# baldhat/yolov10-3D

Hardware: AMD Instinct MI355X
Metric: train_images_per_sec (higher is better)
Workload: dtype bf16

## Files before the change

yolov10-3d_amd/csrc/conv3x3_wgrad_tile.hip:

```cpp
#include "common.h"
#include <cstdlib>

namespace {

__device__ uint4 y3d_wg_zero_page[4];

struct WG3P {
  const void* x;
  const void* dy;
  float* slab;
  long xsb, xsh, xsw, dsw;
  int B, H, W;
  int Cg, Cn, G;
  int ntx, nty;
  int ntiles, tiles_per_split, nslab;
};

typedef __attribute__((ext_vector_type(8))) short s16x8_t;

template <int OFF>
__device__ __forceinline__ s16x4_t ds_tr16(unsigned a) {
  s16x4_t v;
#ifdef Y3D_WGP_NOLDS
  asm volatile("" : "=v"(v) : "v"(a));
  return v;
#endif
  asm volatile("ds_read_b64_tr_b16 %0, %1 offset:%2" : "=v"(v) : "v"(a), "n"(OFF));
  return v;
}
template <int N>
__device__ __forceinline__ void lds_wait(s16x4_t& a, s16x4_t& b, s16x4_t& c, s16x4_t& d) {
  asm volatile("s_waitcnt lgkmcnt(%4)" : "+v"(a), "+v"(b), "+v"(c), "+v"(d) : "n"(N));
}

template <int N>
__device__ __forceinline__ void lds_wait8(s16x4_t& a, s16x4_t& b, s16x4_t& c, s16x4_t& d, s16x4_t& e, s16x4_t& f, s16x4_t& g, s16x4_t& h) {
  asm volatile("s_waitcnt lgkmcnt(%8)" : "+v"(a), "+v"(b), "+v"(c), "+v"(d), "+v"(e), "+v"(f), "+v"(g), "+v"(h) : "n"(N));
}

template <int TH>
__global__ __launch_bounds__(512) void conv3x3_wgrad_tile_kernel(WG3P p) {
  typedef bf16_t T;
  constexpr int NT = 512;
  constexpr int NPX = TH * 16;
  constexpr int HWD = 18;
  constexpr int NPIXH = (TH + 2) * HWD;
  constexpr int DR = NPX * 16 / NT;
  constexpr int HCH = NPIXH * 8;
  constexpr int HR = (HCH + NT - 1) / NT;
  constexpr int DBYTES = NPX * 256, HBYTES = HR * NT * 16, SBYTES = DBYTES + HBYTES;
  extern __shared__ __attribute__((aligned(16))) char smem[];

  const int tid = threadIdx.x, lane = tid & 63, wave = tid >> 6;
  const int wi = wave >> 1, wj = wave & 1;
  const int g = blockIdx.z, split = blockIdx.y;
  const int slab_i = blockIdx.x % p.nslab, cot = blockIdx.x / p.nslab;
  const int c0 = cot * 128, ci0 = slab_i * 64;
  const T* __restrict__ X = (const T*)p.x;
  const T* __restrict__ D = (const T*)p.dy;
  const T* zero = (const T*)y3d_wg_zero_page;

  int d_row[DR], d_px[DR], d_c[DR];
#pragma unroll
  for (int rd = 0; rd < DR; ++rd) {
    int chunk = rd * NT + tid;
    int pp = chunk >> 4, s = chunk & 15;
    d_row[rd] = pp >> 4;
    d_px[rd] = pp & 15;
    d_c[rd] = (s ^ ((pp & 7) << 1)) * 8;
  }
  int h_y[HR], h_x[HR], h_c[HR];
#pragma unroll
  for (int rd = 0; rd < HR; ++rd) {
    int chunk = rd * NT + tid;
    int P = chunk >> 3, s = chunk & 7;
    h_y[rd] = chunk < HCH ? P / HWD : -100000;
    h_x[rd] = P - (P / HWD) * HWD;
    h_c[rd] = (s ^ (((h_x[rd] >> 1) & 3) << 1)) * 8;
  }
  auto issue = [&](int tile, int buf) {
    int tx = tile % p.ntx;
    int t2 = tile / p.ntx;
    int ty = t2 % p.nty;
    int b = t2 / p.nty;
    const int x0 = tx * 16, y0 = ty * TH;
    char* db = smem + buf * SBYTES;
    char* hb = db + DBYTES;
#pragma unroll
    for (int rd = 0; rd < DR; ++rd) {
      int xx = x0 + d_px[rd];
      bool ok = xx < p.W && c0 + d_c[rd] < p.Cn;
      const T* src = ok ? D + (((long)b * p.H + y0 + d_row[rd]) * p.W + xx) * p.dsw + (long)g * p.Cn + c0 + d_c[rd] : zero;
#ifndef Y3D_WGP_NODMA
      __builtin_amdgcn_global_load_lds((const __attribute__((address_space(1))) void*)src,
                                       (__attribute__((address_space(3))) void*)(db + (rd * NT + wave * 64) * 16), 16, 0, 0);
#else
      asm volatile("" ::"v"(src));
#endif
    }
#pragma unroll
    for (int rd = 0; rd < HR; ++rd) {
      if (rd * NT + tid < HCH) {
        int yy = y0 + h_y[rd] - 1, xx = x0 + h_x[rd] - 1;
        bool ok = yy >= 0 && yy < p.H && xx >= 0 && xx < p.W && ci0 + h_c[rd] < p.Cg;
        const T* src = ok ? X + (long)b * p.xsb + (long)yy * p.xsh + (long)xx * p.xsw + (long)g * p.Cg + ci0 + h_c[rd] : zero;
#ifndef Y3D_WGP_NODMA
        __builtin_amdgcn_global_load_lds((const __attribute__((address_space(1))) void*)src,
                                         (__attribute__((address_space(3))) void*)(hb + (rd * NT + wave * 64) * 16), 16, 0, 0);
#else
        asm volatile("" ::"v"(src));
#endif
      }
    }
  };

  f32x4_t acc[9][2][2];
#pragma unroll
  for (int t = 0; t < 9; ++t)
#pragma unroll
    for (int a = 0; a < 2; ++a)
#pragma unroll
      for (int c = 0; c < 2; ++c) acc[t][a][c] = (f32x4_t){0.f, 0.f, 0.f, 0.f};

  const int t_beg = split * p.tiles_per_split;
  const int t_end = min(p.ntiles, t_beg + p.tiles_per_split);
  const int grp = lane >> 4, li = lane & 15, qq = li >> 2, pp4 = li & 3;

  unsigned aoff[2], boff[3][2];
  {
    const int px8 = 4 * grp + qq;
#pragma unroll
    for (int mt = 0; mt < 2; ++mt) {
      const int cch = ((wi * 32 + mt * 16) >> 3) + (pp4 >> 1);
      aoff[mt] = px8 * 256 + ((cch ^ ((px8 & 7) << 1)) << 4) + (pp4 & 1) * 8;
    }
#pragma unroll
    for (int q = 0; q < 3; ++q)
#pragma unroll
      for (int nt = 0; nt < 2; ++nt) {
        const int x = px8 + q;
        const int cch = ((wj * 32 + nt * 16) >> 3) + (pp4 >> 1);
        boff[q][nt] = x * 128 + ((cch ^ (((x >> 1) & 3) << 1)) << 4) + (pp4 & 1) * 8;
      }
  }
  const unsigned smem_base = (unsigned)(size_t)(__attribute__((address_space(3))) const char*)smem;

  if (t_beg < t_end) issue(t_beg, 0);
  asm volatile("s_waitcnt vmcnt(0)" ::: "memory");
  __syncthreads();
  for (int tile = t_beg; tile < t_end; ++tile) {
    const int cur = (tile - t_beg) & 1;
    if (tile + 1 < t_end) issue(tile + 1, cur ^ 1);
#pragma unroll
    for (int ks = 0; ks < NPX / 32; ++ks) {
      bf16x8_t fa[2];
      s16x4_t va[2][2];
      const unsigned dks = smem_base + cur * SBYTES + ks * 8192;
      const unsigned hks = smem_base + cur * SBYTES + DBYTES + ks * (2 * HWD * 128);
#pragma unroll
      for (int mt = 0; mt < 2; ++mt) {
        va[mt][0] = ds_tr16<0>(dks + aoff[mt]);
        va[mt][1] = ds_tr16<4096>(dks + aoff[mt]);
      }
      s16x4_t vr[2][2][4];
      auto issue_q = [&](int q, int buf) {
#pragma unroll
        for (int nt = 0; nt < 2; ++nt) {
          const unsigned a = hks + boff[q][nt];
          vr[buf][nt][0] = ds_tr16<0>(a);
          vr[buf][nt][1] = ds_tr16<HWD * 128>(a);
          vr[buf][nt][2] = ds_tr16<2 * HWD * 128>(a);
          vr[buf][nt][3] = ds_tr16<3 * HWD * 128>(a);
        }
      };
      issue_q(0, 0);
      lds_wait<8>(va[0][0], va[0][1], va[1][0], va[1][1]);
#pragma unroll
      for (int mt = 0; mt < 2; ++mt) fa[mt] = __builtin_bit_cast(bf16x8_t, __builtin_shufflevector(va[mt][0], va[mt][1], 0, 1, 2, 3, 4, 5, 6, 7));
#pragma unroll
      for (int q = 0; q < 3; ++q) {
        const int cb = q & 1;
        if (q < 2) {
          issue_q(q + 1, cb ^ 1);
          lds_wait8<8>(vr[cb][0][0], vr[cb][0][1], vr[cb][0][2], vr[cb][0][3], vr[cb][1][0], vr[cb][1][1], vr[cb][1][2], vr[cb][1][3]);
        } else {
          lds_wait8<0>(vr[cb][0][0], vr[cb][0][1], vr[cb][0][2], vr[cb][0][3], vr[cb][1][0], vr[cb][1][1], vr[cb][1][2], vr[cb][1][3]);
        }
#pragma unroll
        for (int r = 0; r < 3; ++r) {
          bf16x8_t fb[2];
#pragma unroll
          for (int nt = 0; nt < 2; ++nt)
            fb[nt] = __builtin_bit_cast(bf16x8_t, __builtin_shufflevector(vr[cb][nt][r], vr[cb][nt][r + 1], 0, 1, 2, 3, 4, 5, 6, 7));
#pragma unroll
          for (int mt = 0; mt < 2; ++mt)
#pragma unroll
            for (int nt = 0; nt < 2; ++nt)
#ifndef Y3D_WGP_NOMFMA
              acc[r * 3 + q][mt][nt] = __builtin_amdgcn_mfma_f32_16x16x32_bf16(fa[mt], fb[nt], acc[r * 3 + q][mt][nt], 0, 0, 0);
#else
              asm volatile("" ::"v"(fa[mt]), "v"(fb[nt]));
#endif
        }
      }
    }
    asm volatile("s_waitcnt vmcnt(0)" ::: "memory");
    __syncthreads();
  }

  const int Ktot = 9 * p.Cg;
  float* slab = p.slab + ((long)split * p.G * p.Cn + (long)g * p.Cn) * Ktot;
#pragma unroll
  for (int tap = 0; tap < 9; ++tap)
#pragma unroll
    for (int mt = 0; mt < 2; ++mt)
#pragma unroll
      for (int nt = 0; nt < 2; ++nt) {
        int ci = ci0 + wj * 32 + nt * 16 + (lane & 15);
#pragma unroll
        for (int rg = 0; rg < 4; ++rg) {
          int co = c0 + wi * 32 + mt * 16 + (lane >> 4) * 4 + rg;
          if (co < p.Cn && ci < p.Cg) slab[(long)co * Ktot + tap * p.Cg + ci] = acc[tap][mt][nt][rg];
        }
      }
}

template <int TH>
int launch_wg(const WG3P& p, int nsplit, hipStream_t st) {
  constexpr int NPX = TH * 16;
  constexpr int HCH = (TH + 2) * 18 * 8;
  constexpr int HR = (HCH + 511) / 512;
  size_t sm = 2 * ((size_t)NPX * 256 + (size_t)HR * 512 * 16);
  static bool attr_set = false;
  if (!attr_set) {
    (void)hipFuncSetAttribute((const void*)conv3x3_wgrad_tile_kernel<TH>, hipFuncAttributeMaxDynamicSharedMemorySize, (int)sm);
    attr_set = true;
  }
  dim3 grid(p.nslab * cdiv(p.Cn, 128), nsplit, p.G);
  hipLaunchKernelGGL((conv3x3_wgrad_tile_kernel<TH>), grid, dim3(512), sm, st, p);
  Y3D_LAUNCH_CHECK();
  return Y3D_OK;
}

}

int y3d_wgrad_tile_height(int dtype, int H, int W, int Cg, int Cn, int kh, int kw, int stride, int pad) {
  if (dtype != Y3D_BF16 || kh != 3 || kw != 3 || stride != 1 || pad != 1) return 0;
  if (Cg % 16 != 0 || Cg < 64 || Cn % 8 != 0 || W < 8) return 0;
  if (H % 8 == 0) return 8;
  if (H % 4 == 0) return 4;
  return 0;
}

int y3d_wgrad_tile_splits(int th, int B, int H, int W, int Cg, int Cn, int G) {
  long ntiles = (long)B * (H / th) * cdiv(W, 16);
  long blocks = (long)cdiv(Cg, 64) * cdiv(Cn, 128) * G;
  const int target8 = 256;
  const long tgt = th == 8 ? target8 : 2 * target8;
  long want = tgt / blocks;
  if (want > ntiles) want = ntiles;
  long slab_bytes = (long)G * Cn * 9 * Cg * 4;
  long cap = (64L << 20) / slab_bytes;
  if (cap < 16) cap = 16;
  if (cap > 256) cap = 256;
  if (want > cap) want = cap;
  if (want < 1) want = 1;
  return (int)want;
}

int y3d_conv3x3_wgrad_tile_launch(int th, const void* x, long xsb, long xsh, long xsw, const void* dy, long dsw, int B, int H, int W, int Cg,
                                  int Cn, int G, float* slab, int nsplit, void* stream) {
  WG3P p;
  p.x = x; p.dy = dy; p.slab = slab;
  p.xsb = xsb; p.xsh = xsh; p.xsw = xsw; p.dsw = dsw;
  p.B = B; p.H = H; p.W = W; p.Cg = Cg; p.Cn = Cn; p.G = G;
  p.ntx = cdiv(W, 16); p.nty = H / th;
  p.ntiles = B * p.nty * p.ntx;
  p.tiles_per_split = cdiv(p.ntiles, nsplit);
  p.nslab = cdiv(Cg, 64);
  hipStream_t st = (hipStream_t)stream;
  if (th == 8) return launch_wg<8>(p, nsplit, st);
  return launch_wg<4>(p, nsplit, st);
}
```

yolov10-3d_amd/csrc/conv_gemm.hip:

```cpp
#include "common.h"
#include "conv_frag.h"
#include <cstdlib>

namespace {

struct ConvP {
  const void* x;
  const void* w;
  const float* bias;
  const float* scale;
  const float* shift;
  int act;
  void* y;
  float* part;
  long xsb, xsh, xsw;
  long ysw;
  int B, Hg, Wg;
  int Hq, Wq;
  int Cg, Cn, G;
  int kh, kw, stride, pad;
  int Ktot, Kpad;
  int M;
  int ntx, nty;
};
// ... 216 lines not shown
      for (int j = 0; j < 4; ++j) {
        float u = acc[a][b][j] + bv[j];
        if (p.scale) { u = u * sv[j] + hv[j]; if (p.act) u = silu_f(u); }
        v[j] = TT<T>::rnd(u);
        ssum[a][j] += v[j];
        ssq[a][j] += v[j] * v[j];
      }
      if (m < Mc) {
        T* dst = Y + opix * p.ysw + (long)g * p.Cn + co;
        if (co + 3 < p.Cn && ((p.Cn | p.ysw) & 3) == 0) {
          if (sizeof(T) == 2) {
            uint2 u;
            u.x = (unsigned)f2bf(v[0]) | ((unsigned)f2bf(v[1]) << 16);
            u.y = (unsigned)f2bf(v[2]) | ((unsigned)f2bf(v[3]) << 16);
            *(uint2*)dst = u;
          } else {
            *(float4*)dst = make_float4(v[0], v[1], v[2], v[3]);
          }
        } else {
#pragma unroll
          for (int j = 0; j < 4; ++j) if (co + j < p.Cn) TT<T>::st(dst + j, v[j]);
        }
      }
    }
  }
  if (p.part) {
    float* red = (float*)smem;
#pragma unroll
    for (int a = 0; a < TC; ++a)
#pragma unroll
      for (int j = 0; j < 4; ++j) {
        float s = wave_xor_sum16(ssum[a][j]);
        float q = wave_xor_sum16(ssq[a][j]);
        if (lp == 0) {
          int cl = wc * (BC / WC) + a * 16 + lc + j;
          red[(wp * BC + cl) * 2 + 0] = s;
          red[(wp * BC + cl) * 2 + 1] = q;
        }
      }
    __syncthreads();
    if (tid < BC && c0 + tid < p.Cn) {
      float s = 0.f, q = 0.f;
#pragma unroll
      for (int w = 0; w < WP; ++w) { s += red[(w * BC + tid) * 2]; q += red[(w * BC + tid) * 2 + 1]; }
      float* dst = p.part + ((long)tile_x * (p.G * p.Cn) + g * p.Cn + c0 + tid) * 2;
      dst[0] = s;
      dst[1] = q;
    }
  }
}

struct WgradP {
  const void* x;
  const void* dy;
  float* slab;
  long xsb, xsh, xsw;
  long dsw;
  int B, H, W, Ho, Wo;
  int Cg, Cn, G;
  int kh, kw, stride, pad;
  int Ktot, M, nsplit, chunk_px;
};

template <typename T, int W> struct TFrag;
template <int W> struct TFrag<bf16_t, W> {
  typedef bf16x8_t type;
  static constexpr int KSUB_PX = 32;
  static constexpr int PITCH = W * 2 + 32;
  __device__ static __forceinline__ type load(const char* tile, int i0, int k0, int lane) {
    int grp = lane >> 4, li = lane & 15;
    int q = li >> 2, pp = li & 3;
    const char* a0 = tile + (k0 + 4 * grp + q) * PITCH + (i0 + 4 * pp) * 2;
    s16x4_t lo = __builtin_amdgcn_ds_read_tr16_b64_v4i16((s16x4_t __attribute__((address_space(3)))*)(a0));
    s16x4_t hi = __builtin_amdgcn_ds_read_tr16_b64_v4i16((s16x4_t __attribute__((address_space(3)))*)(a0 + 16 * PITCH));
    typedef __attribute__((ext_vector_type(8))) short s16x8_t;
    s16x8_t v = __builtin_shufflevector(lo, hi, 0, 1, 2, 3, 4, 5, 6, 7);
    return __builtin_bit_cast(bf16x8_t, v);
  }
  __device__ static __forceinline__ f32x4_t mma(type a, type b, f32x4_t c) {
    return __builtin_amdgcn_mfma_f32_16x16x32_bf16(a, b, c, 0, 0, 0);
  }
};
template <int W> struct TFrag<float, W> {
  typedef float type;
  static constexpr int KSUB_PX = 4;
  static constexpr int PITCH = W * 4 + 64;
  __device__ static __forceinline__ type load(const char* tile, int i0, int k0, int lane) {
    return *(const float*)(tile + (k0 + (lane >> 4)) * PITCH + (i0 + (lane & 15)) * 4);
  }
  __device__ static __forceinline__ f32x4_t mma(type a, type b, f32x4_t c) {
    return __builtin_amdgcn_mfma_f32_16x16x4f32(a, b, c, 0, 0, 0);
  }
};

template <typename T, int WD, int WX>
__global__ __launch_bounds__(256) void conv_wgrad_kernel(WgradP p) {
  constexpr int CE = TT<T>::CE;
  constexpr int BPK = TT<T>::BKE;
  constexpr int PD = TFrag<T, WD>::PITCH, PX = TFrag<T, WX>::PITCH;
  constexpr int CPD = WD * sizeof(T) / 16, CPX = WX * sizeof(T) / 16;
  constexpr int ND = BPK * CPD / 256 > 0 ? BPK * CPD / 256 : 1;
  constexpr int NX = BPK * CPX / 256 > 0 ? BPK * CPX / 256 : 1;
  constexpr int TA = WD / 32, TB = WX / 32;
  extern __shared__ __attribute__((aligned(16))) char smem[];
  char* sD = smem;
  char* sX = smem + 2 * BPK * PD;

  const int tid = threadIdx.x, lane = tid & 63, wave = tid >> 6;
  const int wi = wave >> 1, wj = wave & 1;
  const int g = blockIdx.z % p.G;
  const int split = blockIdx.z / p.G;
  const int j0 = blockIdx.x * WX;
  const int i0 = blockIdx.y * WD;
  const T* __restrict__ X = (const T*)p.x;
  const T* __restrict__ D = (const T*)p.dy;

  const int mbeg = split * p.chunk_px;
  const int mend = min(p.M, mbeg + p.chunk_px);
  const int nsteps = (mend - mbeg + BPK - 1) / BPK;

  const int ccd = tid % CPD, rd0 = tid / CPD;
  const int ccx = tid % CPX, rx0 = tid / CPX;
  constexpr int RSD = 256 / CPD, RSX = 256 / CPX;
  const bool tdv = BPK * CPD >= 256 || tid < BPK * CPD, txv = BPK * CPX >= 256 || tid < BPK * CPX;
  const int kx = j0 + ccx * CE;
  const bool kx_ok = txv && kx < p.Ktot;
  int tap = 0, ci = 0, tr = 0, tq = 0;
  if (kx_ok) { tap = kx / p.Cg; ci = kx - tap * p.Cg; tr = tap / p.kw; tq = tap - tr * p.kw; }
  const int cd = i0 + ccd * CE;
  const bool cd_ok = tdv && cd < p.Cn;
  const int HW = p.Ho * p.Wo;

  uint4 rd[ND], rx[NX];
  int rb_[NX], rh_[NX], rw_[NX];
#pragma unroll
  for (int i = 0; i < NX; ++i) {
    int m = mbeg + rx0 + RSX * i;
    int b = m / HW;
    int rem = m - b * HW;
    rb_[i] = b;
    rh_[i] = rem / p.Wo;
    rw_[i] = rem - rh_[i] * p.Wo;
  }
  const T* dcol = D + (long)g * p.Cn + cd;
  const T* xcol = X + (long)g * p.Cg + ci + (long)(tr - p.pad) * p.xsh + (long)(tq - p.pad) * p.xsw;
  auto gload = [&](int st) {
#pragma unroll
    for (int i = 0; i < ND; ++i) {
      int m = mbeg + st * BPK + rd0 + RSD * i;
      uint4 vd = make_uint4(0, 0, 0, 0);
      if (m < mend && cd_ok) vd = *(const uint4*)(dcol + (long)m * p.dsw);
      rd[i] = vd;
    }
#pragma unroll
    for (int i = 0; i < NX; ++i) {
      int m = mbeg + st * BPK + rx0 + RSX * i;
      uint4 vx = make_uint4(0, 0, 0, 0);
      if (m < mend && kx_ok) {
        int hh = rh_[i] * p.stride - p.pad + tr, ww = rw_[i] * p.stride - p.pad + tq;
        if (hh >= 0 && ww >= 0 && hh < p.H && ww < p.W)
          vx = *(const uint4*)(xcol + (long)rb_[i] * p.xsb + (long)(rh_[i] * p.stride) * p.xsh + (long)(rw_[i] * p.stride) * p.xsw);
      }
      rx[i] = vx;
      rw_[i] += BPK;
      while (rw_[i] >= p.Wo) { rw_[i] -= p.Wo; ++rh_[i]; }
      while (rh_[i] >= p.Ho) { rh_[i] -= p.Ho; ++rb_[i]; }
    }
  };
  auto lstore = [&](int buf) {
    if (tdv) {
#pragma unroll
      for (int i = 0; i < ND; ++i) *(uint4*)(sD + buf * BPK * PD + (rd0 + RSD * i) * PD + ccd * 16) = rd[i];
    }
    if (txv) {
#pragma unroll
      for (int i = 0; i < NX; ++i) *(uint4*)(sX + buf * BPK * PX + (rx0 + RSX * i) * PX + ccx * 16) = rx[i];
    }
  };

  f32x4_t acc[TA][TB];
#pragma unroll
  for (int a = 0; a < TA; ++a)
#pragma unroll
    for (int b = 0; b < TB; ++b) acc[a][b] = (f32x4_t){0.f, 0.f, 0.f, 0.f};

  if (nsteps > 0) {
    gload(0);
    lstore(0);
  }
  __syncthreads();
  for (int st = 0; st < nsteps; ++st) {
    const int cur = st & 1;
    if (st + 1 < nsteps) gload(st + 1);
    const char* tD = sD + cur * BPK * PD;
    const char* tX = sX + cur * BPK * PX;
#pragma unroll
    for (int k0 = 0; k0 < BPK; k0 += TFrag<T, WD>::KSUB_PX) {
      typename TFrag<T, WD>::type fa[TA], fb[TB];
#pragma unroll
      for (int a = 0; a < TA; ++a) fa[a] = TFrag<T, WD>::load(tD, wi * (WD / 2) + a * 16, k0, lane);
#pragma unroll
      for (int b = 0; b < TB; ++b) fb[b] = TFrag<T, WX>::load(tX, wj * (WX / 2) + b * 16, k0, lane);
#pragma unroll
      for (int a = 0; a < TA; ++a)
#pragma unroll
        for (int b = 0; b < TB; ++b) acc[a][b] = TFrag<T, WD>::mma(fa[a], fb[b], acc[a][b]);
    }
    if (st + 1 < nsteps) lstore(cur ^ 1);
    __syncthreads();
  }
  float* slab = p.slab + ((long)split * p.G * p.Cn + (long)g * p.Cn) * p.Ktot;
#pragma unroll
  for (int a = 0; a < TA; ++a)
#pragma unroll
    for (int b = 0; b < TB; ++b) {
      int k = j0 + wj * (WX / 2) + b * 16 + (lane & 15);
#pragma unroll
      for (int r = 0; r < 4; ++r) {
        int co = i0 + wi * (WD / 2) + a * 16 + (lane >> 4) * 4 + r;
        if (co < p.Cn && k < p.Ktot) slab[(long)co * p.Ktot + k] = acc[a][b][r];
      }
    }
}

template <int SL>
__global__ __launch_bounds__(256) void wgrad_reduce_kernel(const float* __restrict__ slab, float* __restrict__ grad, int nsplit, int Ctot,
                                                           int taps, int Cg, int Cg_real, int accumulate) {
  constexpr int GPB = 256 / SL;
  __shared__ float4 sh[SL][GPB];
  const int e = threadIdx.x % GPB, sl = threadIdx.x / GPB;
  const long idx = ((long)blockIdx.x * GPB + e) * 4;
  const long n = (long)Ctot * taps * Cg;
  float4 s = make_float4(0.f, 0.f, 0.f, 0.f);
  if (idx < n) {
    float4 s0 = s, s1 = s, s2 = s, s3 = s;
    auto add = [](float4& a, const float4 b) { a.x += b.x; a.y += b.y; a.z += b.z; a.w += b.w; };
    int k = sl;
    for (; k + 3 * SL < nsplit; k += 4 * SL) {
      const float4 v0 = *(const float4*)(slab + (long)k * n + idx), v1 = *(const float4*)(slab + (long)(k + SL) * n + idx);
      const float4 v2 = *(const float4*)(slab + (long)(k + 2 * SL) * n + idx), v3 = *(const float4*)(slab + (long)(k + 3 * SL) * n + idx);
      add(s0, v0); add(s1, v1); add(s2, v2); add(s3, v3);
    }
    for (; k < nsplit; k += SL) add(s0, *(const float4*)(slab + (long)k * n + idx));
    s.x = (s0.x + s1.x) + (s2.x + s3.x); s.y = (s0.y + s1.y) + (s2.y + s3.y);
    s.z = (s0.z + s1.z) + (s2.z + s3.z); s.w = (s0.w + s1.w) + (s2.w + s3.w);
  }
  if (SL > 1) {
    sh[sl][e] = s;
    __syncthreads();
    if (sl != 0) return;
#pragma unroll
    for (int j = 1; j < SL; ++j) { const float4 v = sh[j][e]; s.x += v.x; s.y += v.y; s.z += v.z; s.w += v.w; }
  }
  if (idx >= n) return;
  const int ci = (int)(idx % Cg);
  const int tap = (int)((idx / Cg) % taps);
  const int co = (int)(idx / ((long)Cg * taps));
  const float v[4] = {s.x, s.y, s.z, s.w};
#pragma unroll
  for (int j = 0; j < 4; ++j) {
    if (ci + j >= Cg_real) break;
    const long o = ((long)co * Cg_real + ci + j) * taps + tap;
    grad[o] = accumulate ? grad[o] + v[j] : v[j];
  }
}

template <int SL>
__global__ __launch_bounds__(256) void wgrad_reduce_scalar_kernel(const float* __restrict__ slab, float* __restrict__ grad, int nsplit, int Ctot,
                                                           int taps, int Cg, int Cg_real, int accumulate) {
  constexpr int EPB = 256 / SL;
  __shared__ float sh[SL][EPB];
  const int e = threadIdx.x % EPB, sl = threadIdx.x / EPB;
  long idx = (long)blockIdx.x * EPB + e;
  long n = (long)Ctot * taps * Cg;
  float s = 0.f;
  if (idx < n) {
    float s0 = 0.f, s1 = 0.f, s2 = 0.f, s3 = 0.f;
    int k = sl;
    for (; k + 3 * SL < nsplit; k += 4 * SL) {
      s0 += slab[(long)k * n + idx];
      s1 += slab[(long)(k + SL) * n + idx];
      s2 += slab[(long)(k + 2 * SL) * n + idx];
      s3 += slab[(long)(k + 3 * SL) * n + idx];
    }
    for (; k < nsplit; k += SL) s0 += slab[(long)k * n + idx];
    s = (s0 + s1) + (s2 + s3);
  }
  if (SL > 1) {
    sh[sl][e] = s;
    __syncthreads();
    if (sl != 0) return;
#pragma unroll
    for (int j = 1; j < SL; ++j) s += sh[j][e];
  }
  if (idx >= n) return;
  int ci = idx % Cg;
  int tap = (idx / Cg) % taps;
  int co = idx / ((long)Cg * taps);
  if (ci >= Cg_real) return;
  long o = ((long)co * Cg_real + ci) * taps + tap;
  grad[o] = accumulate ? grad[o] + s : s;
}

inline void launch_wgrad_reduce(const float* slab, float* grad, int nsplit, int Ctot, int taps, int Cg, int Cg_real, int accumulate, hipStream_t st) {
  long n = (long)Ctot * taps * Cg;
  long ng = (n + 3) / 4;
  if (n <= 65536 && nsplit >= 64) hipLaunchKernelGGL(wgrad_reduce_kernel<16>, dim3(cdiv(ng, 16)), dim3(256), 0, st, slab, grad, nsplit, Ctot, taps, Cg, Cg_real, accumulate);
  else if (n <= 1048576 && nsplit >= 32) hipLaunchKernelGGL(wgrad_reduce_kernel<8>, dim3(cdiv(ng, 32)), dim3(256), 0, st, slab, grad, nsplit, Ctot, taps, Cg, Cg_real, accumulate);
  else if (nsplit >= 8) hipLaunchKernelGGL(wgrad_reduce_kernel<2>, dim3(cdiv(ng, 128)), dim3(256), 0, st, slab, grad, nsplit, Ctot, taps, Cg, Cg_real, accumulate);
  else hipLaunchKernelGGL(wgrad_reduce_scalar_kernel<1>, dim3(cdiv(n, 256)), dim3(256), 0, st, slab, grad, nsplit, Ctot, taps, Cg, Cg_real, accumulate);
}

template <typename T>
__global__ void pack_w_fwd_kernel(const float* __restrict__ w, T* __restrict__ out, int Cout, int Cg, int Cg_pad, int taps, int Kpad) {
  long idx = (long)blockIdx.x * blockDim.x + threadIdx.x;
  long n = (long)Cout * Kpad;
  if (idx >= n) return;
  int k = idx % Kpad;
  int co = idx / Kpad;
  float v = 0.f;
  if (k < taps * Cg_pad) {
    int tap = k / Cg_pad, ci = k - tap * Cg_pad;
    if (ci < Cg) v = w[((long)co * Cg + ci) * taps + tap];
  }
  TT<T>::st(out + idx, v);
}

template <typename T>
__global__ void pack_w_dgrad_kernel(const float* __restrict__ w, T* __restrict__ out, int G, int Cn, int Cg, int taps, int Kpad) {
  long idx = (long)blockIdx.x * blockDim.x + threadIdx.x;
  long n = (long)G * Cg * Kpad;
  if (idx >= n) return;
  int k = idx % Kpad;
  int ci = (idx / Kpad) % Cg;
  int g = idx / ((long)Kpad * Cg);
  float v = 0.f;
  if (k < taps * Cn) {
    int tap = k / Cn, co = k - tap * Cn;
    v = w[((long)(g * Cn + co) * Cg + ci) * taps + tap];
  }
  TT<T>::st(out + idx, v);
}

template <typename T>
__global__ __launch_bounds__(256) void mt_pack_w_kernel(const long* __restrict__ desc, const int* __restrict__ ctensor, const int* __restrict__ coff,
                                                        int chunk) {
  constexpr int CAP = 4096;
  __shared__ float st[CAP + 64];
  const long* d = desc + (long)ctensor[blockIdx.x] * 8;
  const float* __restrict__ w = (const float*)d[0];
  T* __restrict__ out = (T*)d[1];
  const int a = (int)d[2], b = (int)d[3], c = (int)d[4], taps = (int)d[5], Kpad = (int)d[6], mode = (int)d[7];
  const long n = mode == 0 ? (long)a * Kpad : (long)a * c * Kpad;
  const long beg = (long)coff[blockIdx.x] * chunk;
  const long end = beg + chunk < n ? beg + chunk : n;
  const int tid = threadIdx.x;
  const long rb = beg / Kpad, re = (end - 1) / Kpad;
  if (mode == 0) {
    for (long idx = beg + tid; idx < end; idx += 256) {
      const int k = (int)(idx % Kpad), co = (int)(idx / Kpad);
      float v = 0.f;
      if (k < taps * c) {
        const int tap = k / c, ci = k - tap * c;
        if (ci < b) v = w[((long)co * b + ci) * taps + tap];
      }
      TT<T>::st(out + idx, v);
    }
  } else {
    const int CB = b < 256 ? b : 256;
    int R = CAP / (taps * (CB + 1));
    if (R < 1) R = 1;
    const int P = CB + 1;
    for (long r0 = rb; r0 <= re;) {
      const int g = (int)(r0 / c), ci0 = (int)(r0 - (long)g * c);
      int nr = R;
      if (nr > c - ci0) nr = c - ci0;
      if (nr > re - r0 + 1) nr = (int)(re - r0 + 1);
      const int seg = nr * taps;
      for (int co0 = 0; co0 < b; co0 += CB) {
        const int cb = b - co0 < CB ? b - co0 : CB;
        __syncthreads();
        for (int i = tid; i < cb * seg; i += 256) {
          const int col = i / seg, j = i - col * seg;
          st[j * P + col] = w[((long)(g * b + co0 + col) * c + ci0) * taps + j];
        }
        __syncthreads();
        for (int o = tid; o < seg * cb; o += 256) {
          const int j = o / cb, col = o - j * cb;
          const int cil = j / taps, tap = j - cil * taps;
          const long idx = (r0 + cil) * Kpad + (long)tap * b + co0 + col;
          if (idx >= beg && idx < end) TT<T>::st(out + idx, st[j * P + col]);
        }
      }
      for (int o = tid; o < nr * (Kpad - taps * b); o += 256) {
        const int rl = o / (Kpad - taps * b), k = taps * b + o - rl * (Kpad - taps * b);
        const long idx = (r0 + rl) * Kpad + k;
        if (idx >= beg && idx < end) TT<T>::st(out + idx, 0.f);
      }
      r0 += nr;
    }
  }
}

template <typename T, int MODE>
int launch_conv_mode(ConvP p, hipStream_t st) {
  dim3 block(256);
  const unsigned ny = MODE == 2 ? 4 : 1;
  p.ntx = MODE == 2 ? cdiv((long)p.B * ((p.Hq + 1) / 2) * ((p.Wq + 1) / 2), 128) : cdiv(p.M, 128);
  const long t128 = (long)p.ntx * cdiv(p.Cn, 128) * ny * p.G;
  int bc = p.Cn > 64 ? 128 : (p.Cn > 32 ? 64 : 32);
  if (p.Cn % 32 == 0) {
    if (bc == 128 && t128 < 192) bc = 64;
    if (bc == 64 && (long)p.ntx * cdiv(p.Cn, 64) * ny * p.G < 192 && p.Cn > 32) bc = 32;
  }
  p.nty = cdiv(p.Cn, bc);
  if (bc == 128) {
    size_t sm = 2 * (128 + 128) * 128;
    hipLaunchKernelGGL((conv_gemm_kernel<T, 128, 128, 2, 2, MODE>), dim3(p.ntx * p.nty, ny, p.G), block, sm, st, p);
  } else if (bc == 64) {
    size_t sm = 2 * (128 + 64) * 128;
    hipLaunchKernelGGL((conv_gemm_kernel<T, 128, 64, 4, 1, MODE>), dim3(p.ntx * p.nty, ny, p.G), block, sm, st, p);
  } else {
    size_t sm = 2 * (128 + 32) * 128;
    hipLaunchKernelGGL((conv_gemm_kernel<T, 128, 32, 4, 1, MODE>), dim3(p.ntx * p.nty, ny, p.G), block, sm, st, p);
  }
  Y3D_LAUNCH_CHECK();
  return Y3D_OK;
}

template <typename T, bool DGRAD>
int launch_conv(ConvP p, hipStream_t st) {
  if (DGRAD && p.kh == 3 && p.kw == 3 && p.stride == 2 && p.pad == 1 && p.Cg % TT<T>::CE == 0) return launch_conv_mode<T, 2>(p, st);
  return launch_conv_mode<T, DGRAD ? 1 : 0>(p, st);
}

}

int y3d_conv3x3_tile_route(int dtype, int B, int H, int W, int Cg, int Cn, int G, int kh, int kw, int stride, int pad);
int y3d_conv3x3_flat_tiles(int B, int H, int W);
int y3d_conv3x3_tile_launch(int dtype, int route, const void* x, long xsb, long xsh, long xsw, int B, int H, int W, int Cg, int Cn, int G,
                            const void* w, int Ktot, void* y, long ysw, float* part, int flip, const float* scale, const float* shift, int act,
                            void* stream);

int y3d_wgrad_tile_height(int dtype, int H, int W, int Cg, int Cn, int kh, int kw, int stride, int pad);
int y3d_wgrad_tile_splits(int th, int B, int H, int W, int Cg, int Cn, int G);
int y3d_conv3x3_wgrad_tile_launch(int th, const void* x, long xsb, long xsh, long xsw, const void* dy, long dsw, int B, int H, int W, int Cg,
                                  int Cn, int G, float* slab, int nsplit, void* stream);

int y3d_conv1x1_stream_ok(int dtype, long M, int K, int N, long xsw, int G = 1);
int y3d_conv1x1_stream_launch(const void* x, long xsw, const void* w, int Kpad, const float* bias, const float* scale, const float* shift, int act,
                              void* y, long ysw, float* part, long M, int K, int N, int G, void* stream);
int y3d_wgrad1x1_stream_ok(int dtype, long M, int Cg, int Cn, long xsw, long dsw);
int y3d_wgrad1x1_stream_launch(const void* x, long xsw, const void* dy, long dsw, long M, int Cg, int Cn, float* slab, int nsplit, int chunk_px,
                               void* stream);
int y3d_conv3x3s2_dgrad_ok(int dtype, int B, int Ho, int Wo, int H, int W, int Cout, int Cin, long dsw, long xsw);
int y3d_conv3x3s2_dgrad_launch(const void* dy, long dsw, int B, int Ho, int Wo, int Cout, const void* w_packed_dgrad, int Kpad, void* dx, long xsw,
                               int H, int W, int Cin, void* stream);
int y3d_conv3x3_small_ok(int dtype, int B, int H, int W, int Cin, int Cout, int rows);
int y3d_conv3x3_small_launch(const void* x, long xsb, long xsh, long xsw, int B, int H, int W, int Cin, int Cout, const void* w, int Ktot, void* y,
                             long ysw, float* part, int rows, int flip, const float* scale, const float* shift, int act, const void* res, long rsw,
                             void* stream);
int y3d_conv3x3_small_rows(int B, int H, int W, int Cin, int Cout);
int y3d_conv3x3_small_s2_ok(int dtype, int B, int H, int W, int Cin, int Cout);
int y3d_conv3x3_small_s2_rows(int B, int H, int W, int Cin, int Cout);
int y3d_conv3x3_small_s2_launch(const void* x, long xsb, long xsh, long xsw, int B, int H, int W, int Cin, int Cout, const void* w, int Ktot, void* y,
                                long ysw, float* part, int rows, const float* scale, const float* shift, int act, void* stream);
int y3d_conv1x1_stream_rows(long M, int K, int N, int G = 1);
int y3d_wgrad3x3_small_ok(int dtype, int B, int H, int W, int Cin, int Cout);
int y3d_wgrad3x3_small_splits(int B, int H, int W);
int y3d_wgrad3x3_small_launch(const void* x, long xsb, long xsh, long xsw, const void* dy, long dsw, int B, int H, int W, int Cin, int Cout,
                              float* slab, int nsplit, void* stream);
static inline bool dense_pixels(int B, int H, int W, long sb, long sh, long sw) {
  return (H == 1 || sh == (long)W * sw) && (B == 1 || sb == (long)H * W * sw);
}

static int g_tile_kernels = 1;
extern "C" int y3d_conv2d_wgrad_splits(int dtype, int B, int Ho, int Wo, int Cout, int Cin_g, int groups, int kh, int kw);

static int conv_route(int dtype, int op, int epi, int B, int H, int W, int Ho, int Wo, int Cin, int Cout, int groups, int kh, int kw, int stride,
                      int pad, bool dense, long asw, long bsw, bool cin_full) {
  const int ce = dtype == Y3D_BF16 ? 8 : 4;
  const bool k1 = kh == 1 && kw == 1 && stride == 1 && pad == 0, k3s1 = kh == 3 && kw == 3 && stride == 1 && pad == 1,
             k3s2 = kh == 3 && kw == 3 && stride == 2 && pad == 1;
  if (op == Y3D_OP_FWD) {
    Y3D_CHECK(dtype == Y3D_BF16 || dtype == Y3D_F32, "conv2d_fwd: bad dtype %d", dtype);
    Y3D_CHECK(B > 0 && H > 0 && W > 0 && Cin > 0 && Cout > 0 && groups > 0, "conv2d_fwd: empty shape");
    Y3D_CHECK(Cin % groups == 0 && Cout % groups == 0, "conv2d_fwd: channels not divisible by groups");
    Y3D_CHECK((Cin / groups) % ce == 0, "conv2d_fwd: Cin/groups=%d must be a multiple of %d (pad the input)", Cin / groups, ce);
    Y3D_CHECK(kh * kw <= 64, "conv2d_fwd: at most 64 filter taps");
    Y3D_CHECK(epi >= Y3D_EPI_RAW && epi <= Y3D_EPI_BIAS, "conv2d_fwd: bad epilogue %d", epi);
    const int Cg = Cin / groups, Cn = Cout / groups;
    const long M = (long)B * Ho * Wo;
    const bool bias = epi == Y3D_EPI_BIAS;
    if (k1 && dense && y3d_conv1x1_stream_ok(dtype, M, Cg, Cn, asw, groups)) return Y3D_ROUTE_STREAM1X1;
    Y3D_CHECK(!(epi == Y3D_EPI_PARTIALS && k1 && y3d_conv1x1_stream_ok(dtype, M, Cg, Cn, Cin, groups)),
              "conv2d_fwd: 1x1 input view must be pixel-dense and below 4 GB for the BatchNorm partial layout of this shape");
    if (k3s1 && groups == 1 && !bias && y3d_conv3x3_small_ok(dtype, B, H, W, Cin, Cout, 1)) return Y3D_ROUTE_SMALL;
    Y3D_CHECK(epi != Y3D_EPI_AFFINE_RES, "conv2d_fwd_affine_res: no kernel with a residual epilogue takes this geometry (ask y3d_conv2d_fwd_affine_res_ok first)");
    if (k3s2 && groups == 1 && !bias && y3d_conv3x3_small_s2_ok(dtype, B, H, W, Cin, Cout)) return Y3D_ROUTE_SMALL_S2;
    if (!bias && g_tile_kernels) return y3d_conv3x3_tile_route(dtype, B, H, W, Cg, Cn, groups, kh, kw, stride, pad);
    return Y3D_ROUTE_GENERIC;
  }
  if (op == Y3D_OP_BWD_DATA) {
    Y3D_CHECK(dtype == Y3D_BF16 || dtype == Y3D_F32, "conv2d_bwd_data: bad dtype %d", dtype);
    Y3D_CHECK(groups > 0 && Cin % groups == 0 && Cout % groups == 0, "conv2d_bwd_data: channels not divisible by groups");
    Y3D_CHECK((Cout / groups) % ce == 0, "conv2d_bwd_data: Cout/groups=%d must be a multiple of %d", Cout / groups, ce);
    Y3D_CHECK(kh * kw <= 64, "conv2d_bwd_data: at most 64 filter taps");
    Y3D_CHECK(epi == 0, "conv2d_bwd_data: no epilogue variants");
    const int Cg = Cout / groups, Cn = Cin / groups;
    if (k1 && dense && y3d_conv1x1_stream_ok(dtype, (long)B * H * W, Cg, Cn, asw, groups)) return Y3D_ROUTE_STREAM1X1;
    if (k3s1 && groups == 1 && Ho == H && Wo == W && y3d_conv3x3_small_ok(dtype, B, H, W, Cout, Cin, 1)) return Y3D_ROUTE_SMALL;
    if (k3s2 && groups == 1 && dense && y3d_conv3x3s2_dgrad_ok(dtype, B, Ho, Wo, H, W, Cout, Cin, asw, bsw)) return Y3D_ROUTE_S2_DGRAD;
    if (g_tile_kernels && Ho == H && Wo == W) return y3d_conv3x3_tile_route(dtype, B, H, W, Cg, Cn, groups, kh, kw, stride, pad);
    return Y3D_ROUTE_GENERIC;
  }
  Y3D_CHECK(op == Y3D_OP_BWD_WEIGHT, "conv2d_route: bad op %d", op);
  Y3D_CHECK(dtype == Y3D_BF16 || dtype == Y3D_F32, "conv2d_bwd_weight: bad dtype %d", dtype);
  Y3D_CHECK(groups > 0 && Cin % groups == 0 && Cout % groups == 0, "conv2d_bwd_weight: channels not divisible by groups");
  Y3D_CHECK((Cin / groups) % ce == 0 && (Cout / groups) % ce == 0, "conv2d_bwd_weight: per-group channels must be multiples of %d", ce);
  Y3D_CHECK(epi == 0, "conv2d_bwd_weight: no epilogue variants");
  if (k3s1 && groups == 1 && cin_full && y3d_wgrad3x3_small_ok(dtype, B, H, W, Cin, Cout)) return Y3D_ROUTE_WGRAD_SMALL;
  if (g_tile_kernels && cin_full && y3d_wgrad_tile_height(dtype, H, W, Cin / groups, Cout / groups, kh, kw, stride, pad)) return Y3D_ROUTE_WGRAD_TILE;
  if (k1 && groups == 1 && cin_full && dense && y3d_wgrad1x1_stream_ok(dtype, (long)B * Ho * Wo, Cin, Cout, asw, bsw)) return Y3D_ROUTE_WGRAD_STREAM1X1;
  return Y3D_ROUTE_GENERIC;
}

extern "C" {

int y3d_get_tile_kernels(void) { return g_tile_kernels; }

int y3d_set_tile_kernels(int enable) {
  int old = g_tile_kernels;
  g_tile_kernels = enable ? 1 : 0;
  return old;
}

int y3d_conv_stat_blocks(int B, int Ho, int Wo) { return cdiv((long)B * Ho * Wo, 128); }

int y3d_conv2d_route(int dtype, int op, int epi, int B, int H, int W, int Cin, int Cout, int groups, int kh, int kw, int stride, int pad) {
  Y3D_CHECK(kh > 0 && kw > 0 && stride > 0 && pad >= 0, "conv2d_route: bad filter geometry");
  const int Ho = (H + 2 * pad - kh) / stride + 1, Wo = (W + 2 * pad - kw) / stride + 1;
  Y3D_CHECK(Ho > 0 && Wo > 0, "conv2d_route: empty output");
  if (op == Y3D_OP_BWD_DATA) return conv_route(dtype, op, epi, B, H, W, Ho, Wo, Cin, Cout, groups, kh, kw, stride, pad, true, Cout, Cin, true);
  return conv_route(dtype, op, epi, B, H, W, Ho, Wo, Cin, Cout, groups, kh, kw, stride, pad, true, Cin, Cout, true);
}

int y3d_conv2d_wgrad_plan(int dtype, int B, int H, int W, int Cin, int Cout, int groups, int kh, int kw, int stride, int pad) {
  int Ho = (H + 2 * pad - kh) / stride + 1, Wo = (W + 2 * pad - kw) / stride + 1;
  switch (conv_route(dtype, Y3D_OP_BWD_WEIGHT, 0, B, H, W, Ho, Wo, Cin, Cout, groups, kh, kw, stride, pad, true, Cin, Cout, true)) {
    case Y3D_ROUTE_WGRAD_SMALL: return y3d_wgrad3x3_small_splits(B, H, W);
    case Y3D_ROUTE_WGRAD_TILE:
      return y3d_wgrad_tile_splits(y3d_wgrad_tile_height(dtype, H, W, Cin / groups, Cout / groups, kh, kw, stride, pad), B, H, W, Cin / groups,
                                   Cout / groups, groups);
    case Y3D_ROUTE_WGRAD_STREAM1X1: {
      const int target = 256;
      const long tiles = (long)cdiv(Cin, Cin <= 64 ? 64 : 128) * cdiv(Cout, Cout <= 64 ? 64 : 128);
      long want = target / tiles, maxs = cdiv((long)B * H * W, 4 * 64);
      if (want > maxs) want = maxs;
      return (int)(want < 1 ? 1 : want);
    }
    default: return y3d_conv2d_wgrad_splits(dtype, B, Ho, Wo, Cout, Cin / groups, groups, kh, kw);
  }
}

int y3d_conv2d_stat_rows(int dtype, int B, int H, int W, int Cin, int Cout, int groups, int kh, int kw, int stride, int pad) {
  int Ho = (H + 2 * pad - kh) / stride + 1, Wo = (W + 2 * pad - kw) / stride + 1;
  switch (conv_route(dtype, Y3D_OP_FWD, Y3D_EPI_PARTIALS, B, H, W, Ho, Wo, Cin, Cout, groups, kh, kw, stride, pad, true, Cin, Cout, true)) {
    case Y3D_ROUTE_STREAM1X1: return y3d_conv1x1_stream_rows((long)B * H * W, Cin / groups, Cout / groups, groups);
    case Y3D_ROUTE_SMALL: return y3d_conv3x3_small_rows(B, H, W, Cin, Cout);
    case Y3D_ROUTE_SMALL_S2: return y3d_conv3x3_small_s2_rows(B, H, W, Cin, Cout);
    case Y3D_ROUTE_FLAT: return y3d_conv3x3_flat_tiles(B, H, W);
    case Y3D_ROUTE_TILE8: case Y3D_ROUTE_WIDE3_8: return B * cdiv(H, 8) * cdiv(W, 16);
    case Y3D_ROUTE_TILE16: case Y3D_ROUTE_WIDE3_16: return B * cdiv(H, 16) * cdiv(W, 16);
    default: return cdiv((long)B * Ho * Wo, 128);
  }
}

int y3d_conv_kpad(int dtype, int k_total) {
  int ce = dtype == Y3D_BF16 ? 8 : 4;
  return cdiv(k_total, ce) * ce;
}

int y3d_pack_weight_fwd(int dtype, const float* w_oihw, void* out, int Cout, int Cin_g, int Cin_g_pad, int kh, int kw, void* stream) {
  int ce = dtype == Y3D_BF16 ? 8 : 4;
  Y3D_CHECK(Cin_g_pad >= Cin_g && Cin_g_pad % ce == 0, "pack_weight_fwd: Cin_g_pad=%d must be a multiple of %d", Cin_g_pad, ce);
  int taps = kh * kw, Kpad = taps * Cin_g_pad;
  long n = (long)Cout * Kpad;
  hipStream_t st = (hipStream_t)stream;
  if (dtype == Y3D_BF16)
    hipLaunchKernelGGL(pack_w_fwd_kernel<bf16_t>, dim3(cdiv(n, 256)), dim3(256), 0, st, w_oihw, (bf16_t*)out, Cout, Cin_g, Cin_g_pad, taps, Kpad);
  else
    hipLaunchKernelGGL(pack_w_fwd_kernel<float>, dim3(cdiv(n, 256)), dim3(256), 0, st, w_oihw, (float*)out, Cout, Cin_g, Cin_g_pad, taps, Kpad);
  Y3D_LAUNCH_CHECK();
  return Y3D_OK;
}

int y3d_pack_weight_dgrad(int dtype, const float* w_oihw, void* out, int Cout, int Cin_g, int groups, int kh, int kw, void* stream) {
  Y3D_CHECK(Cout % groups == 0, "pack_weight_dgrad: Cout %% groups");
  int Cn = Cout / groups, taps = kh * kw;
  int Kpad = y3d_conv_kpad(dtype, taps * Cn);
  long n = (long)groups * Cin_g * Kpad;
  hipStream_t st = (hipStream_t)stream;
  if (dtype == Y3D_BF16)
    hipLaunchKernelGGL(pack_w_dgrad_kernel<bf16_t>, dim3(cdiv(n, 256)), dim3(256), 0, st, w_oihw, (bf16_t*)out, groups, Cn, Cin_g, taps, Kpad);
  else
    hipLaunchKernelGGL(pack_w_dgrad_kernel<float>, dim3(cdiv(n, 256)), dim3(256), 0, st, w_oihw, (float*)out, groups, Cn, Cin_g, taps, Kpad);
  Y3D_LAUNCH_CHECK();
  return Y3D_OK;
}

static int check_align(const char* what, const void* ptr, long s0, long s1, long s2, int ce) {
  Y3D_CHECK(((uintptr_t)ptr & 15) == 0, "%s: pointer not 16-byte aligned", what);
// ... 202 lines not shown
```

Baseline: 1441.

## Retile 3x3 wgrad waves to 2x4 and add row-wise split-K reduce kernel

The 3x3 weight-gradient tile kernel changes its wave layout from 4x2 to 2x4. Each wave now owns 64 output channels by 16 input channels, so it loads four A fragments and one B fragment set instead of two and two. This cuts the per-tap halo LDS transpose reads, at the cost of more A reads and a different register footprint. Separately, a new reduce kernel sums split-K slabs per output-channel row into shared memory, then writes the permuted weight layout contiguously, replacing scattered strided writes for large reductions.

```diff
diff --git a/yolov10-3d_amd/csrc/conv3x3_wgrad_tile.hip b/yolov10-3d_amd/csrc/conv3x3_wgrad_tile.hip
--- a/yolov10-3d_amd/csrc/conv3x3_wgrad_tile.hip
+++ b/yolov10-3d_amd/csrc/conv3x3_wgrad_tile.hip
@@ -52,7 +52,7 @@
   extern __shared__ __attribute__((aligned(16))) char smem[];
 
   const int tid = threadIdx.x, lane = tid & 63, wave = tid >> 6;
-  const int wi = wave >> 1, wj = wave & 1;
+  const int wi = wave >> 2, wj = wave & 3;
   const int g = blockIdx.z, split = blockIdx.y;
   const int slab_i = blockIdx.x % p.nslab, cot = blockIdx.x / p.nslab;
   const int c0 = cot * 128, ci0 = slab_i * 64;
@@ -114,34 +114,30 @@
     }
   };
 
-  f32x4_t acc[9][2][2];
+  f32x4_t acc[9][4];
 #pragma unroll
   for (int t = 0; t < 9; ++t)
 #pragma unroll
-    for (int a = 0; a < 2; ++a)
-#pragma unroll
-      for (int c = 0; c < 2; ++c) acc[t][a][c] = (f32x4_t){0.f, 0.f, 0.f, 0.f};
+    for (int a = 0; a < 4; ++a) acc[t][a] = (f32x4_t){0.f, 0.f, 0.f, 0.f};
 
   const int t_beg = split * p.tiles_per_split;
   const int t_end = min(p.ntiles, t_beg + p.tiles_per_split);
   const int grp = lane >> 4, li = lane & 15, qq = li >> 2, pp4 = li & 3;
 
-  unsigned aoff[2], boff[3][2];
+  unsigned aoff[4], boff[3];
   {
     const int px8 = 4 * grp + qq;
 #pragma unroll
-    for (int mt = 0; mt < 2; ++mt) {
-      const int cch = ((wi * 32 + mt * 16) >> 3) + (pp4 >> 1);
+    for (int mt = 0; mt < 4; ++mt) {
+      const int cch = ((wi * 64 + mt * 16) >> 3) + (pp4 >> 1);
       aoff[mt] = px8 * 256 + ((cch ^ ((px8 & 7) << 1)) << 4) + (pp4 & 1) * 8;
     }
 #pragma unroll
-    for (int q = 0; q < 3; ++q)
-#pragma unroll
-      for (int nt = 0; nt < 2; ++nt) {
-        const int x = px8 + q;
-        const int cch = ((wj * 32 + nt * 16) >> 3) + (pp4 >> 1);
-        boff[q][nt] = x * 128 + ((cch ^ (((x >> 1) & 3) << 1)) << 4) + (pp4 & 1) * 8;
-      }
+    for (int q = 0; q < 3; ++q) {
+      const int x = px8 + q;
+      const int cch = ((wj * 16) >> 3) + (pp4 >> 1);
+      boff[q] = x * 128 + ((cch ^ (((x >> 1) & 3) << 1)) << 4) + (pp4 & 1) * 8;
+    }
   }
   const unsigned smem_base = (unsigned)(size_t)(__attribute__((address_space(3))) const char*)smem;
 
@@ -153,53 +149,45 @@
     if (tile + 1 < t_end) issue(tile + 1, cur ^ 1);
 #pragma unroll
     for (int ks = 0; ks < NPX / 32; ++ks) {
-      bf16x8_t fa[2];
-      s16x4_t va[2][2];
+      bf16x8_t fa[4];
+      s16x4_t va[4][2];
       const unsigned dks = smem_base + cur * SBYTES + ks * 8192;
       const unsigned hks = smem_base + cur * SBYTES + DBYTES + ks * (2 * HWD * 128);
 #pragma unroll
-      for (int mt = 0; mt < 2; ++mt) {
+      for (int mt = 0; mt < 4; ++mt) {
         va[mt][0] = ds_tr16<0>(dks + aoff[mt]);
         va[mt][1] = ds_tr16<4096>(dks + aoff[mt]);
       }
-      s16x4_t vr[2][2][4];
+      s16x4_t vr[2][4];
       auto issue_q = [&](int q, int buf) {
-#pragma unroll
-        for (int nt = 0; nt < 2; ++nt) {
-          const unsigned a = hks + boff[q][nt];
-          vr[buf][nt][0] = ds_tr16<0>(a);
-          vr[buf][nt][1] = ds_tr16<HWD * 128>(a);
-          vr[buf][nt][2] = ds_tr16<2 * HWD * 128>(a);
-          vr[buf][nt][3] = ds_tr16<3 * HWD * 128>(a);
-        }
+        const unsigned a = hks + boff[q];
+        vr[buf][0] = ds_tr16<0>(a);
+        vr[buf][1] = ds_tr16<HWD * 128>(a);
+        vr[buf][2] = ds_tr16<2 * HWD * 128>(a);
+        vr[buf][3] = ds_tr16<3 * HWD * 128>(a);
       };
       issue_q(0, 0);
-      lds_wait<8>(va[0][0], va[0][1], va[1][0], va[1][1]);
-#pragma unroll
-      for (int mt = 0; mt < 2; ++mt) fa[mt] = __builtin_bit_cast(bf16x8_t, __builtin_shufflevector(va[mt][0], va[mt][1], 0, 1, 2, 3, 4, 5, 6, 7));
+      lds_wait8<4>(va[0][0], va[0][1], va[1][0], va[1][1], va[2][0], va[2][1], va[3][0], va[3][1]);
+#pragma unroll
+      for (int mt = 0; mt < 4; ++mt) fa[mt] = __builtin_bit_cast(bf16x8_t, __builtin_shufflevector(va[mt][0], va[mt][1], 0, 1, 2, 3, 4, 5, 6, 7));
 #pragma unroll
       for (int q = 0; q < 3; ++q) {
         const int cb = q & 1;
         if (q < 2) {
           issue_q(q + 1, cb ^ 1);
-          lds_wait8<8>(vr[cb][0][0], vr[cb][0][1], vr[cb][0][2], vr[cb][0][3], vr[cb][1][0], vr[cb][1][1], vr[cb][1][2], vr[cb][1][3]);
+          lds_wait<4>(vr[cb][0], vr[cb][1], vr[cb][2], vr[cb][3]);
         } else {
-          lds_wait8<0>(vr[cb][0][0], vr[cb][0][1], vr[cb][0][2], vr[cb][0][3], vr[cb][1][0], vr[cb][1][1], vr[cb][1][2], vr[cb][1][3]);
+          lds_wait<0>(vr[cb][0], vr[cb][1], vr[cb][2], vr[cb][3]);
         }
 #pragma unroll
         for (int r = 0; r < 3; ++r) {
-          bf16x8_t fb[2];
-#pragma unroll
-          for (int nt = 0; nt < 2; ++nt)
-            fb[nt] = __builtin_bit_cast(bf16x8_t, __builtin_shufflevector(vr[cb][nt][r], vr[cb][nt][r + 1], 0, 1, 2, 3, 4, 5, 6, 7));
-#pragma unroll
-          for (int mt = 0; mt < 2; ++mt)
-#pragma unroll
-            for (int nt = 0; nt < 2; ++nt)
+          const bf16x8_t fb = __builtin_bit_cast(bf16x8_t, __builtin_shufflevector(vr[cb][r], vr[cb][r + 1], 0, 1, 2, 3, 4, 5, 6, 7));
+#pragma unroll
+          for (int mt = 0; mt < 4; ++mt)
 #ifndef Y3D_WGP_NOMFMA
-              acc[r * 3 + q][mt][nt] = __builtin_amdgcn_mfma_f32_16x16x32_bf16(fa[mt], fb[nt], acc[r * 3 + q][mt][nt], 0, 0, 0);
+            acc[r * 3 + q][mt] = __builtin_amdgcn_mfma_f32_16x16x32_bf16(fa[mt], fb, acc[r * 3 + q][mt], 0, 0, 0);
 #else
-              asm volatile("" ::"v"(fa[mt]), "v"(fb[nt]));
+            asm volatile("" ::"v"(fa[mt]), "v"(fb));
 #endif
         }
       }
@@ -213,16 +201,14 @@
 #pragma unroll
   for (int tap = 0; tap < 9; ++tap)
 #pragma unroll
-    for (int mt = 0; mt < 2; ++mt)
-#pragma unroll
-      for (int nt = 0; nt < 2; ++nt) {
-        int ci = ci0 + wj * 32 + nt * 16 + (lane & 15);
-#pragma unroll
-        for (int rg = 0; rg < 4; ++rg) {
-          int co = c0 + wi * 32 + mt * 16 + (lane >> 4) * 4 + rg;
-          if (co < p.Cn && ci < p.Cg) slab[(long)co * Ktot + tap * p.Cg + ci] = acc[tap][mt][nt][rg];
-        }
-      }
+    for (int mt = 0; mt < 4; ++mt) {
+      int ci = ci0 + wj * 16 + (lane & 15);
+#pragma unroll
+      for (int rg = 0; rg < 4; ++rg) {
+        int co = c0 + wi * 64 + mt * 16 + (lane >> 4) * 4 + rg;
+        if (co < p.Cn && ci < p.Cg) slab[(long)co * Ktot + tap * p.Cg + ci] = acc[tap][mt][rg];
+      }
+    }
 }
 
 template <int TH>
diff --git a/yolov10-3d_amd/csrc/conv_gemm.hip b/yolov10-3d_amd/csrc/conv_gemm.hip
--- a/yolov10-3d_amd/csrc/conv_gemm.hip
+++ b/yolov10-3d_amd/csrc/conv_gemm.hip
@@ -542,12 +542,50 @@
   grad[o] = accumulate ? grad[o] + s : s;
 }
 
+constexpr int WGRAD_ROW_MAX = 4608;
+template <int SL>
+__global__ __launch_bounds__(256) void wgrad_reduce_rows_kernel(const float* __restrict__ slab, float* __restrict__ grad, int nsplit, int Ctot,
+                                                                int taps, int Cg, int Cg_real, int accumulate) {
+  __shared__ float row[WGRAD_ROW_MAX];
+  const int co = blockIdx.x, nr = taps * Cg;
+  const long n = (long)Ctot * nr;
+  const float* src = slab + (long)co * nr;
+  auto add = [](float4& a, const float4 b) { a.x += b.x; a.y += b.y; a.z += b.z; a.w += b.w; };
+  for (int i = threadIdx.x * 4; i < nr; i += 1024) {
+    float4 s = make_float4(0.f, 0.f, 0.f, 0.f);
+#pragma unroll
+    for (int sl = 0; sl < SL; ++sl) {
+      float4 s0 = make_float4(0.f, 0.f, 0.f, 0.f), s1 = s0, s2 = s0, s3 = s0;
+      int k = sl;
+      for (; k + 3 * SL < nsplit; k += 4 * SL) {
+        const float4 v0 = *(const float4*)(src + (long)k * n + i), v1 = *(const float4*)(src + (long)(k + SL) * n + i);
+        const float4 v2 = *(const float4*)(src + (long)(k + 2 * SL) * n + i), v3 = *(const float4*)(src + (long)(k + 3 * SL) * n + i);
+        add(s0, v0); add(s1, v1); add(s2, v2); add(s3, v3);
+      }
+      for (; k < nsplit; k += SL) add(s0, *(const float4*)(src + (long)k * n + i));
+      const float4 r = make_float4((s0.x + s1.x) + (s2.x + s3.x), (s0.y + s1.y) + (s2.y + s3.y), (s0.z + s1.z) + (s2.z + s3.z),
+                                   (s0.w + s1.w) + (s2.w + s3.w));
+      if (sl == 0) s = r; else add(s, r);
+    }
+    const int tap = i / Cg, ci = i - tap * Cg;
+    const float v[4] = {s.x, s.y, s.z, s.w};
+#pragma unroll
+    for (int j = 0; j < 4; ++j) row[(ci + j) * taps + tap] = v[j];
+  }
+  __syncthreads();
+  float* dst = grad + (long)co * Cg_real * taps;
+  for (int j = threadIdx.x; j < Cg_real * taps; j += 256) dst[j] = accumulate ? dst[j] + row[j] : row[j];
+}
+
 inline void launch_wgrad_reduce(const float* slab, float* grad, int nsplit, int Ctot, int taps, int Cg, int Cg_real, int accumulate, hipStream_t st) {
   long n = (long)Ctot * taps * Cg;
   long ng = (n + 3) / 4;
+  const bool rows = taps > 1 && Cg % 4 == 0 && taps * Cg <= WGRAD_ROW_MAX;
   if (n <= 65536 && nsplit >= 64) hipLaunchKernelGGL(wgrad_reduce_kernel<16>, dim3(cdiv(ng, 16)), dim3(256), 0, st, slab, grad, nsplit, Ctot, taps, Cg, Cg_real, accumulate);
   else if (n <= 1048576 && nsplit >= 32) hipLaunchKernelGGL(wgrad_reduce_kernel<8>, dim3(cdiv(ng, 32)), dim3(256), 0, st, slab, grad, nsplit, Ctot, taps, Cg, Cg_real, accumulate);
+  else if (nsplit >= 8 && rows) hipLaunchKernelGGL(wgrad_reduce_rows_kernel<2>, dim3(Ctot), dim3(256), 0, st, slab, grad, nsplit, Ctot, taps, Cg, Cg_real, accumulate);
   else if (nsplit >= 8) hipLaunchKernelGGL(wgrad_reduce_kernel<2>, dim3(cdiv(ng, 128)), dim3(256), 0, st, slab, grad, nsplit, Ctot, taps, Cg, Cg_real, accumulate);
+  else if (rows) hipLaunchKernelGGL(wgrad_reduce_rows_kernel<1>, dim3(Ctot), dim3(256), 0, st, slab, grad, nsplit, Ctot, taps, Cg, Cg_real, accumulate);
   else hipLaunchKernelGGL(wgrad_reduce_scalar_kernel<1>, dim3(cdiv(n, 256)), dim3(256), 0, st, slab, grad, nsplit, Ctot, taps, Cg, Cg_real, accumulate);
 }
 
```

After: 1454, median of 6. No clear change (+0.9%).
